# TJUMMG/OCPG

Hardware: AMD Instinct MI355X
Metric: clips/sec fwd+bwd (5x384x640, R101) (higher is better)
Workload: dtype bf16

## Files before the change

include/ocpg_hip.h:

```cpp
#ifndef OCPG_HIP_H
#define OCPG_HIP_H
#include <stdint.h>

#ifdef __cplusplus
extern "C" {
#endif

int ocpg_msda_fwd_f32(const float* value, const int64_t* shapes, const int64_t* level_start,
                      const float* loc, const float* attn,
                      int N, int S, int M, int D, int L, int Lq, int P,
                      float* out, const int64_t* shapes_host, void* stream);
int ocpg_msda_fwd_f64(const double* value, const int64_t* shapes, const int64_t* level_start,
                      const double* loc, const double* attn,
                      int N, int S, int M, int D, int L, int Lq, int P,
                      double* out, void* stream);

int ocpg_msda_bwd_f32(const float* value, const int64_t* shapes, const int64_t* level_start,
                      const float* loc, const float* attn, const float* grad_out,
                      int N, int S, int M, int D, int L, int Lq, int P,
                      float* grad_value, float* grad_loc, float* grad_attn,
                      const int64_t* shapes_host, void* stream);
int ocpg_msda_bwd_value_f32(const float* loc, const float* attn, const float* grad_out,
                            int N, int S, int M, int D, int L, int Lq, int P,
                            float* grad_value, const int64_t* shapes_host, void* stream);
int ocpg_msda_bwd_locattn_f32(const float* value, const int64_t* shapes, const int64_t* level_start,
                              const float* loc, const float* attn, const float* grad_out,
                              int N, int S, int M, int D, int L, int Lq, int P,
                              float* grad_loc, float* grad_attn, void* stream);
int ocpg_msda_fused_fwd_f32(const float* value, const int64_t* shapes, const int64_t* level_start,
                            const float* qproj, const float* ref,
                            int N, int S, int M, int D, int L, int Lq, int P,
                            float* out, float* loc_out, float* attn_out, void* stream);
int ocpg_msda_fused_bwd_qproj_f32(const float* value, const int64_t* shapes, const int64_t* level_start,
                                  const float* loc, const float* attn, const float* grad_out,
                                  int N, int S, int M, int D, int L, int Lq, int P,
                                  float* grad_qproj, void* stream);
int ocpg_msda_bwd_value_sel_f32(const float* loc, const float* attn, const float* grad_out,
                                int N, int S, int M, int D, int L, int Lq, int P,
                                float* grad_value, const int64_t* shapes_host, int* sel_state, void* stream);
int ocpg_msda_bwd_f64(const double* value, const int64_t* shapes, const int64_t* level_start,
                      const double* loc, const double* attn, const double* grad_out,
                      int N, int S, int M, int D, int L, int Lq, int P,
                      double* grad_value, double* grad_loc, double* grad_attn, void* stream);

int ocpg_msda_fwd_h16(const void* value, const int64_t* shapes, const int64_t* level_start,
                      const float* loc, const float* attn,
                      int N, int S, int M, int D, int L, int Lq, int P,
                      void* out, const int64_t* shapes_host, int dtype, void* stream);
int ocpg_msda_bwd_h16(const void* value, const int64_t* shapes, const int64_t* level_start,
                      const float* loc, const float* attn, const void* grad_out,
                      int N, int S, int M, int D, int L, int Lq, int P,
                      float* grad_value, float* grad_loc, float* grad_attn,
                      const int64_t* shapes_host, int* sel_state, int dtype, void* stream);
int ocpg_msda_bwd_value_h16(const float* loc, const float* attn, const void* grad_out,
                            int N, int S, int M, int D, int L, int Lq, int P,
                            float* grad_value, const int64_t* shapes_host, int* sel_state, int dtype, void* stream);
int ocpg_msda_bwd_locattn_h16(const void* value, const int64_t* shapes, const int64_t* level_start,
                              const float* loc, const float* attn, const void* grad_out,
                              int N, int S, int M, int D, int L, int Lq, int P,
                              float* grad_loc, float* grad_attn, int dtype, void* stream);
int ocpg_msda_fused_fwd_h16(const void* value, const int64_t* shapes, const int64_t* level_start,
                            const float* qproj, const float* ref,
                            int N, int S, int M, int D, int L, int Lq, int P,
                            void* out, float* loc_out, float* attn_out, int dtype, void* stream);
int ocpg_msda_fused_bwd_qproj_h16(const void* value, const int64_t* shapes, const int64_t* level_start,
                                  const float* loc, const float* attn, const void* grad_out,
                                  int N, int S, int M, int D, int L, int Lq, int P,
                                  float* grad_qproj, int dtype, void* stream);

int ocpg_bn_act_fwd(const void* x, const float* scale, const float* shift, const void* skip, void* y,
                    long long n_outer, int C, long long inner, int relu, int dtype, void* stream);
int ocpg_bn_act_bwd(const void* gy, const void* y, const float* scale, void* gx, void* gskip,
                    long long n_outer, int C, long long inner, int relu, int dtype, void* stream);

int ocpg_gemm_dgrad_bn_tile(long long M, int N, int K);
int ocpg_gemm_dgrad_bn(const void* a, const void* w, const void* c, const void* mask, const float* scale, void* out, void* out_skip,
                       long long M, int N, int K, int dtype, int tile, void* stream);

int ocpg_win_attn_fwd(const void* qkv, const float* biasT, const int* region, float scale, int BW, int NW, int N, int H,
                      int head_dim, void* out, float* lse, int dtype, void* stream);
int ocpg_win_attn_bwd(const void* qkv, const float* bias, const float* biasT, const int* region, float scale, int BW, int NW,
                      int N, int H, int head_dim, const void* out, const void* dout, const float* lse, void* dqkv, float* Dbuf,
                      float* dbiasT, int dtype, void* stream);

int ocpg_win_attn_bwd_mfma(const void* qkv, const float* bias, const float* biasT, const int* region, float scale, int BW, int NW, int N,
                           int H, int head_dim, const void* out, const void* dout, const float* lse, void* dqkv, float* Dbuf, void* dS,
                           int dtype, void* stream);

int ocpg_win_attn_dtable_supported(int N, int head_dim, int dtype, int T);
int ocpg_win_attn_bwd_mfma_dtable(const void* qkv, const float* bias, const float* biasT, const int* region, float scale, int BW, int NW,
                                  int N, int H, int head_dim, const void* out, const void* dout, const float* lse, void* dqkv, float* Dbuf,
                                  const int* tok_code, int code_off, int T, float* partials, float* dtable, int dtype, void* stream);

int ocpg_dynmask_fwd_f32(const float* feats, const float* params, const float* refpix, int BT, int Q, int C, int H, int W,
                         int stride, float* out, float* pre1, void* stream);

int ocpg_dynmask_bwd_pre_f32(const float* dout, const float* pre1, const float* params, int BT, int Q, int C, int H, int W,
                             int stride, float* dpre, float* part, float* w0d, void* stream);
int ocpg_dynmask_bwd_fin_f32(const float* part, const float* params, const float* refpix, const float* dw0, int BT, int Q, int C,
                             int H, int W, float* dparams, float* dref, void* stream);

int ocpg_im2col3x3_nhwc(const void* x, int N, int H, int W, int C, int stride, int dil, void* cols, int dtype, void* stream);
int ocpg_col2im3x3_nhwc(const void* dcols, int N, int H, int W, int C, int stride, int dil, void* dx, int dtype, void* stream);

int ocpg_conv3x3_mfma_fwd(const void* x, const void* w, const float* scale, const float* bias, int relu, int N, int H, int W,
                          int Cin, int Cout, int stride, void* y, void* stream);
int ocpg_conv3x3_mfma_fwd_cols(const void* x, const void* w, const float* scale, const float* bias, int relu, int N, int H, int W, int Cin,
                               int Cout, int stride, void* y, void* cols, void* stream);
int ocpg_conv3x3_mfma_dgrad(const void* dy, const void* wT, int N, int H, int W, int Cin, int Cout, int stride, void* dx,
                            void* stream);
int ocpg_conv3x3_mfma_dgrad_masked(const void* dy, const void* wT, const void* mask_y, const float* scale, int N, int H, int W, int Cin,
                                   int Cout, int stride, void* dx, void* stream);
int ocpg_conv3x3_mfma_dgrad_w(const void* dy, const void* w, const void* mask_y, const float* scale, int N, int H, int W, int Cin, int Cout,
                              int stride, void* dx, void* stream);
int ocpg_conv3x3_mfma_body_splits(long long M, int ncols, int kchannels);
int ocpg_conv3x3_mfma_fwd_bn_splitk(const void* x, const void* w, const float* scale, const float* shift, int relu, int N, int H, int W, int Cin,
                                    int Cout, int stride, int splits, float* part, void* y, void* stream);
int ocpg_conv3x3_mfma_dgrad_w_splitk(const void* dy, const void* w, const void* mask_y, const float* scale, int N, int H, int W, int Cin,
                                     int Cout, int stride, int splits, float* part, void* dx, void* stream);
int ocpg_conv3x3_mfma_wgrad_splits(int N, int H, int W, int Cin, int Cout, int stride);
int ocpg_conv3x3_mfma_wgrad(const void* gz, const void* x, int N, int H, int W, int Cin, int Cout, int stride, void* part, void* stream);
int ocpg_conv3x3_mfma_fwd_cols_h16(const void* x, const void* w, const float* scale, const float* bias, int relu, int N, int H, int W, int Cin,
                                   int Cout, int stride, void* y, void* cols, int dtype, void* stream);
int ocpg_conv3x3_mfma_dgrad_w_h16(const void* dy, const void* w, const void* mask_y, const float* scale, int N, int H, int W, int Cin, int Cout,
                                  int stride, void* dx, int dtype, void* stream);
int ocpg_conv3x3_mfma_wgrad_h16(const void* gz, const void* x, int N, int H, int W, int Cin, int Cout, int stride, void* part, int dtype,
// ... 165 lines not shown
```

ocpg_amd/_lib.py:

```python
import ctypes
import os

import torch

_HERE = os.path.dirname(os.path.abspath(__file__))
LIB_PATH = os.environ.get("OCPG_HIP_LIB") or os.path.join(_HERE, "lib", "libocpg_hip.so")
_lib = None

_i64p = ctypes.c_void_p
_vp = ctypes.c_void_p
_int = ctypes.c_int

SIGNATURES = {
    "ocpg_msda_fwd_f32": [_vp, _i64p, _i64p, _vp, _vp] + [_int] * 7 + [_vp, _vp, _vp],
    "ocpg_msda_fwd_f64": [_vp, _i64p, _i64p, _vp, _vp] + [_int] * 7 + [_vp, _vp],
    "ocpg_msda_bwd_f32": [_vp, _i64p, _i64p, _vp, _vp, _vp] + [_int] * 7 + [_vp, _vp, _vp, _vp, _vp],
    "ocpg_msda_bwd_value_f32": [_vp, _vp, _vp] + [_int] * 7 + [_vp, _vp, _vp],
    "ocpg_msda_fused_fwd_f32": [_vp, _i64p, _i64p, _vp, _vp] + [_int] * 7 + [_vp, _vp, _vp, _vp],
    "ocpg_msda_fused_bwd_qproj_f32": [_vp, _i64p, _i64p, _vp, _vp, _vp] + [_int] * 7 + [_vp, _vp],
    "ocpg_msda_bwd_value_sel_f32": [_vp, _vp, _vp] + [_int] * 7 + [_vp, _vp, _vp, _vp],
    "ocpg_msda_bwd_locattn_f32": [_vp, _i64p, _i64p, _vp, _vp, _vp] + [_int] * 7 + [_vp, _vp, _vp],
    "ocpg_msda_bwd_f64": [_vp, _i64p, _i64p, _vp, _vp, _vp] + [_int] * 7 + [_vp, _vp, _vp, _vp],
    "ocpg_msda_fwd_h16": [_vp, _i64p, _i64p, _vp, _vp] + [_int] * 7 + [_vp, _vp, _int, _vp],
    "ocpg_msda_bwd_h16": [_vp, _i64p, _i64p, _vp, _vp, _vp] + [_int] * 7 + [_vp, _vp, _vp, _vp, _vp, _int, _vp],
    "ocpg_msda_bwd_value_h16": [_vp, _vp, _vp] + [_int] * 7 + [_vp, _vp, _vp, _int, _vp],
    "ocpg_msda_bwd_locattn_h16": [_vp, _i64p, _i64p, _vp, _vp, _vp] + [_int] * 7 + [_vp, _vp, _int, _vp],
    "ocpg_msda_fused_fwd_h16": [_vp, _i64p, _i64p, _vp, _vp] + [_int] * 7 + [_vp, _vp, _vp, _int, _vp],
    "ocpg_msda_fused_bwd_qproj_h16": [_vp, _i64p, _i64p, _vp, _vp, _vp] + [_int] * 7 + [_vp, _int, _vp],
    "ocpg_bn_act_fwd": [_vp, _vp, _vp, _vp, _vp, ctypes.c_longlong, _int, ctypes.c_longlong, _int, _int, _vp],
    "ocpg_bn_act_bwd": [_vp, _vp, _vp, _vp, _vp, ctypes.c_longlong, _int, ctypes.c_longlong, _int, _int, _vp],
    "ocpg_gemm_dgrad_bn_tile": [ctypes.c_longlong, _int, _int],
    "ocpg_gemm_dgrad_bn": [_vp] * 7 + [ctypes.c_longlong, _int, _int, _int, _int, _vp],
    "ocpg_dynmask_fwd_f32": [_vp, _vp, _vp] + [_int] * 6 + [_vp, _vp, _vp],
    "ocpg_dynmask_bwd_pre_f32": [_vp, _vp, _vp] + [_int] * 6 + [_vp, _vp, _vp, _vp],
    "ocpg_dynmask_bwd_fin_f32": [_vp, _vp, _vp, _vp] + [_int] * 5 + [_vp, _vp, _vp],
    "ocpg_conv3x3_mfma_fwd": [_vp, _vp, _vp, _vp] + [_int] * 7 + [_vp, _vp],
    "ocpg_conv3x3_mfma_fwd_cols": [_vp, _vp, _vp, _vp] + [_int] * 7 + [_vp, _vp, _vp],
    "ocpg_conv3x3_mfma_dgrad": [_vp, _vp] + [_int] * 6 + [_vp, _vp],
    "ocpg_conv3x3_mfma_dgrad_masked": [_vp, _vp, _vp, _vp] + [_int] * 6 + [_vp, _vp],
    "ocpg_conv3x3_mfma_dgrad_w": [_vp, _vp, _vp, _vp] + [_int] * 6 + [_vp, _vp],
    "ocpg_conv3x3_mfma_splits": [_int] * 6,
    "ocpg_conv3x3_mfma_wgrad_splits": [_int] * 6,
    "ocpg_conv3x3_mfma_body_splits": [ctypes.c_longlong, _int, _int],
    "ocpg_conv3x3_mfma_fwd_bn_splitk": [_vp, _vp, _vp, _vp] + [_int] * 8 + [_vp, _vp, _vp],
    "ocpg_conv3x3_mfma_dgrad_w_splitk": [_vp, _vp, _vp, _vp] + [_int] * 7 + [_vp, _vp, _vp],
    "ocpg_conv3x3_mfma_wgrad": [_vp, _vp] + [_int] * 6 + [_vp, _vp],
    "ocpg_conv3x3_mfma_fwd_cols_h16": [_vp, _vp, _vp, _vp] + [_int] * 7 + [_vp, _vp, _int, _vp],
    "ocpg_conv3x3_mfma_dgrad_w_h16": [_vp, _vp, _vp, _vp] + [_int] * 6 + [_vp, _int, _vp],
    "ocpg_conv3x3_mfma_wgrad_h16": [_vp, _vp] + [_int] * 6 + [_vp, _int, _vp],
    "ocpg_conv3x3_mfma_dgrad_w_s2": [_vp, _vp, _vp, _vp] + [_int] * 6 + [_vp, _vp],
    "ocpg_conv3x3_mfma_dgrad_w_s2_h16": [_vp, _vp, _vp, _vp] + [_int] * 6 + [_vp, _int, _vp],
    "ocpg_conv3x3_mfma_fwd_splitk": [_vp, _vp, _vp] + [_int] * 7 + [_vp, _vp, _int, _vp, _vp],
    "ocpg_conv3x3_mfma_fwd_splitk_h16": [_vp, _vp, _vp] + [_int] * 7 + [_vp, _vp, _int, _vp, _int, _vp],
    "ocpg_gemm": [_vp, _vp, _vp, _vp] + [_int] * 4 + [ctypes.c_longlong] * 10 + [ctypes.c_float, ctypes.c_float, _vp],
    "ocpg_gemm_plans": [],
    "ocpg_gemm_tuned": [_vp],
    "ocpg_gemm_tune_rejected": [],
    "ocpg_gemm_set_tuning": [_int],
    "ocpg_gemm_export_picks": [_vp, ctypes.c_longlong],
    "ocpg_gemm_import_picks": [_vp, ctypes.c_longlong],
    "ocpg_window_means3x3_fwd": [_vp, ctypes.c_longlong, _int, _int, _int, _vp, _vp],
    "ocpg_window_means3x3_bwd": [_vp, ctypes.c_longlong, _int, _int, _vp, _vp],
    "ocpg_window_sums3x3_cl_bands": [_int],
    "ocpg_window_sums3x3_cl": [_vp, _int, _int, _int, _int, _int, _vp, _vp],
    "ocpg_window_means3x3_bwd_cl": [_vp, _int, _int, _int, _int, _vp, _vp, _vp],
    "ocpg_mso_conv3x3": [_vp, _int, _int, _vp, _int, _vp, _vp, _int, _vp, _int, _vp, _vp, _int] + [_int] * 6 + [_vp],
    "ocpg_mso_wgrad_rows": [_int] * 4,
    "ocpg_mso_wgrad": [_vp, _int, _int, _vp, _vp, _vp] + [_int] * 8 + [_vp],
    "ocpg_bilinear_nhwc_fwd": [_vp] + [_int] * 6 + [_vp, _vp],
    "ocpg_bilinear_nhwc_bwd": [_vp] + [_int] * 6 + [_vp, _vp],
    "ocpg_small_linear_fwd": [_vp, _int, _vp, _vp, _int, _int, _int, _int, _vp, _vp],
    "ocpg_small_linear_bwd": [_vp, _int, _vp, _int, _vp, _vp, _int, _int, _int, _vp, _vp, _vp, _vp],
    "ocpg_small_linear_fwd_h16": [_vp, _int, _vp, _vp, _int, _int, _int, _int, _vp, _int, _vp],
    "ocpg_small_linear_bwd_h16": [_vp, _int, _vp, _int, _vp, _vp, _int, _int, _int, _vp, _vp, _vp, _int, _vp],
    "ocpg_small_linear_f32_fwd": [_vp, _vp, _vp, _int, _int, _int, _vp, _vp],
    "ocpg_small_linear_f32_bwd": [_vp, _vp, _vp, _int, _int, _int, _vp, _vp, _vp, _vp],
    "ocpg_layernorm_blocks": [ctypes.c_longlong],
    "ocpg_groupnorm_cl_work": [ctypes.c_longlong, _int, _int, _int],
    "ocpg_groupnorm_cl_fwd": [_vp, _int, _vp, _vp, ctypes.c_longlong, _int, _int, _int, ctypes.c_float, _vp, _vp, _vp, _vp, _vp],
    "ocpg_groupnorm_cl_bwd": [_vp, _vp, _int, _vp, _vp, _vp, ctypes.c_longlong, _int, _int, _int, _vp, _vp, _vp, _vp],
    "ocpg_groupnorm_cl2cl_fwd": [_vp, _int, _vp, _vp, ctypes.c_longlong, _int, _int, _int, ctypes.c_float, _vp, _vp, _vp, _vp, _vp],
    "ocpg_groupnorm_cl2cl_bwd": [_vp, _vp, _int, _vp, _vp, _vp, ctypes.c_longlong, _int, _int, _int, _vp, _vp, _vp, _vp],
    "ocpg_layernorm_fwd": [_vp, _int, _vp, _vp, ctypes.c_longlong, _int, ctypes.c_float, _vp, _int, _vp, _vp, _vp],
    "ocpg_layernorm_bwd": [_vp, _int, _vp, _int, _vp, _vp, _vp, ctypes.c_longlong, _int, _vp, _int, _vp, _vp, _vp],
    "ocpg_gather_rows_bwd": [_vp, _vp, _vp, _int, _int, _vp, _vp],
    "ocpg_relpos_bias_fwd": [_vp, _vp, _int, ctypes.c_longlong, _int, _vp, _vp, _vp],
    "ocpg_relpos_bias_bwd": [_vp, _vp, _vp, _int, _int, _int, _int, _vp, _vp],
    "ocpg_gather_rows_pad": [_vp, _vp] + [ctypes.c_longlong] * 4 + [_vp, _vp],
    "ocpg_graph_replace_memsets": [_vp, _vp],
    "ocpg_graph_stats": [_vp, _vp],
    "ocpg_graph_memcpy_nodes": [_vp, _vp, _int],
    "ocpg_gemm_bn_act": [_vp] * 6 + [_int, _int] + [ctypes.c_longlong] * 3 + [_vp],
    "ocpg_levelset_fwd_f32": [_vp] * 3 + [_int] * 6 + [_vp] * 4,
    "ocpg_levelset_bwd_f32": [_vp] * 5 + [_int] * 6 + [_vp] * 3,
    "ocpg_proj_fwd_f32": [_vp] * 5 + [_int] * 5 + [_vp] * 5,
    "ocpg_proj_bwd_f32": [_vp] * 9 + [_int] * 5 + [_vp] * 4,
    "ocpg_matcher_cost_f32": [_vp] * 3 + [ctypes.c_longlong] * 4 + [_vp] * 4 + [_int] * 7 + [ctypes.c_float] * 5 + [_vp] * 4,
    "ocpg_dropout_add_ln_fwd": [_vp] * 4 + [ctypes.c_longlong, _int, ctypes.c_float, ctypes.c_float, ctypes.c_ulonglong, ctypes.c_ulonglong, _vp, _int]
                               + [_vp] * 4,
    "ocpg_dropout_add_ln_bwd": [_vp] * 6 + [ctypes.c_longlong, _int, ctypes.c_float, ctypes.c_ulonglong, ctypes.c_ulonglong, _vp, _int] + [_vp] * 4,
    "ocpg_dropout_add_ln_bwd_slots": [ctypes.c_longlong],
    "ocpg_bias_relu_dropout_fwd": [_vp, _vp, ctypes.c_longlong, _int, ctypes.c_float, ctypes.c_ulonglong, ctypes.c_ulonglong, _vp, _int, _vp, _vp],
    "ocpg_bias_relu_dropout_bwd": [_vp, _vp, ctypes.c_longlong, _int, ctypes.c_float, _int, _vp, _vp, _vp],
    "ocpg_bias_relu_dropout_bwd_slots": [ctypes.c_longlong, _int, _int],
    "ocpg_multi_cast": [_vp] * 4 + [_int, ctypes.c_longlong, _int, _int, _vp],
# ... 148 lines not shown
```

ocpg_amd/models/ops/functions/ms_deform_attn_func.py:

```python
import ctypes

import torch
from torch.autograd import Function
from torch.autograd.function import once_differentiable

from ...._lib import check, lib, require_gpu, stream_ptr


_TIMING = {"on": False, "events": []}


def enable_kernel_timing(on=True):
    _TIMING["on"] = on
    _TIMING["events"] = []


def collect_kernel_timing():
    torch.cuda.synchronize()
    out = {}
    for key, e0, e1 in _TIMING["events"]:
        d = out.setdefault(key, {"ms": 0.0, "n": 0})
        d["ms"] += e0.elapsed_time(e1)
        d["n"] += 1
    _TIMING["events"] = []
# ... 187 lines not shown
                    loc = (ref.view(N, Lq, 1, L, 1, 2) + off.reshape(N, Lq, M, L, P, 2)).contiguous()
                    rc = lib().ocpg_msda_fwd_h16(value.data_ptr(), shapes.data_ptr(), level_start.data_ptr(), loc.data_ptr(), attn.data_ptr(),
                                                 N, S, M, D, L, Lq, P, out.data_ptr(), None, code, stream_ptr())
                check(rc, "ocpg_msda_fused_fwd_h16")
            else:
                check(lib().ocpg_msda_fused_fwd_f32(value.data_ptr(), shapes.data_ptr(), level_start.data_ptr(), qproj.data_ptr(), ref.data_ptr(),
                                                    N, S, M, D, L, Lq, P, out.data_ptr(), loc.data_ptr(), attn.data_ptr(), stream_ptr()),
                      "ocpg_msda_fused_fwd")
        ctx.save_for_backward(value, shapes, level_start, loc, attn)
        ctx.shapes_host = getattr(shapes, "_ocpg_host", None)
        ctx.sel_state = sel_state
        ctx.qshape = qproj.shape
        ctx.mark_non_differentiable(loc, attn)
        return out, loc, attn

    @staticmethod
    @once_differentiable
    def backward(ctx, grad_output, _gloc, _gattn):
        value, shapes, level_start, loc, attn = ctx.saved_tensors
        N, S, M, D = value.shape
        _, Lq, _, L, P, _ = loc.shape
        go = grad_output.contiguous()
        hs = ctx.shapes_host if ctx.shapes_host is not None else _host_shapes(shapes)
        if value.dtype in _H16:
            return MSDeformAttnFusedFunction._backward_h16(ctx, value, shapes, level_start, loc, attn, go, hs)
        grad_value = torch.zeros_like(value)
        grad_q = torch.empty(ctx.qshape, dtype=value.dtype, device=value.device)
        L_ = lib()
        with torch.cuda.device(value.device):
            with _timed("bwd_enc_value"):
                args = (loc.data_ptr(), attn.data_ptr(), go.data_ptr(), N, S, M, D, L, Lq, P, grad_value.data_ptr(), ctypes.c_void_p(hs.data_ptr()))
                if ctx.sel_state is not None:
                    rc = L_.ocpg_msda_bwd_value_sel_f32(*args, ctx.sel_state.data_ptr(), stream_ptr())
                else:
                    rc = L_.ocpg_msda_bwd_value_f32(*args, stream_ptr())
            if rc == -2000:
                grad_value.zero_()
                gl, ga = torch.empty_like(loc), torch.empty_like(attn)
                check(L_.ocpg_msda_bwd_f32(value.data_ptr(), shapes.data_ptr(), level_start.data_ptr(), loc.data_ptr(), attn.data_ptr(), go.data_ptr(),
                                           N, S, M, D, L, Lq, P, grad_value.data_ptr(), gl.data_ptr(), ga.data_ptr(), ctypes.c_void_p(hs.data_ptr()),
                                           stream_ptr()), "ocpg_msda_bwd")
                glogit = attn.view(N, Lq, M, L * P) * (ga.view(N, Lq, M, L * P) - (attn * ga).view(N, Lq, M, L * P).sum(-1, keepdim=True))
                grad_q = torch.cat([gl.reshape(N, Lq, -1), glogit.reshape(N, Lq, -1)], -1)
                return grad_value, None, None, grad_q, None, None, None, None
            check(rc, "ocpg_msda_bwd_value")
            with _timed("bwd_enc_locattn"):
                check(L_.ocpg_msda_fused_bwd_qproj_f32(value.data_ptr(), shapes.data_ptr(), level_start.data_ptr(), loc.data_ptr(), attn.data_ptr(),
                                                       go.data_ptr(), N, S, M, D, L, Lq, P, grad_q.data_ptr(), stream_ptr()), "ocpg_msda_fused_bwd_qproj")
        return grad_value, None, None, grad_q, None, None, None, None

    @staticmethod
    def _backward_h16(ctx, value, shapes, level_start, loc, attn, go, hs):
        N, S, M, D = value.shape
        _, Lq, _, L, P, _ = loc.shape
        if go.dtype != value.dtype:
            raise RuntimeError(f"MSDeformAttnFusedFunction: grad_output must have value's dtype {value.dtype} (got {go.dtype})")
        code = _H16[value.dtype]
        grad_value = torch.zeros(value.shape, dtype=torch.float32, device=value.device)
        grad_q = torch.empty(ctx.qshape, dtype=torch.float32, device=value.device)
        sel = ctx.sel_state.data_ptr() if ctx.sel_state is not None else None
        hsp = ctypes.c_void_p(hs.data_ptr())
        L_ = lib()
        with torch.cuda.device(value.device):
            with _timed("bwd_enc_value"):
                rc = L_.ocpg_msda_bwd_value_h16(loc.data_ptr(), attn.data_ptr(), go.data_ptr(), N, S, M, D, L, Lq, P, grad_value.data_ptr(), hsp, sel,
                                                code, stream_ptr())
            if rc == 0:
                with _timed("bwd_enc_locattn"):
                    rc = L_.ocpg_msda_fused_bwd_qproj_h16(value.data_ptr(), shapes.data_ptr(), level_start.data_ptr(), loc.data_ptr(), attn.data_ptr(),
                                                          go.data_ptr(), N, S, M, D, L, Lq, P, grad_q.data_ptr(), code, stream_ptr())
                if rc == -2000:
                    grad_value.zero_()
            if rc == -2000:
                gl, ga = torch.empty_like(loc), torch.empty_like(attn)
                with _timed("bwd_enc"):
                    check(L_.ocpg_msda_bwd_h16(value.data_ptr(), shapes.data_ptr(), level_start.data_ptr(), loc.data_ptr(), attn.data_ptr(), go.data_ptr(),
                                               N, S, M, D, L, Lq, P, grad_value.data_ptr(), gl.data_ptr(), ga.data_ptr(), hsp, sel, code, stream_ptr()),
                          "ocpg_msda_bwd_h16")
                glogit = attn.view(N, Lq, M, L * P) * (ga.view(N, Lq, M, L * P) - (attn * ga).view(N, Lq, M, L * P).sum(-1, keepdim=True))
                grad_q = torch.cat([gl.reshape(N, Lq, -1), glogit.reshape(N, Lq, -1)], -1).view(ctx.qshape)
            else:
                check(rc, "ocpg_msda_fused_bwd_h16")
        return grad_value.to(value.dtype), None, None, grad_q, None, None, None, None
```

ocpg_amd/models/ops/modules/ms_deform_attn.py:

```python
import math
import os
import warnings

import torch
import torch.nn.functional as F
from torch import nn

from ... import amp_cache
from ...amp_cache import TokenLinear, linear
from ....util.misc import memo
from ..functions import MSDeformAttnFunction
from ..functions.ms_deform_attn_func import MSDeformAttnFusedFunction


FUSED_FRONT = os.environ.get("OCPG_MSDA_FUSED_FRONT", "1") != "0"
FUSED_FRONT_H16 = os.environ.get("OCPG_MSDA_FUSED_FRONT_H16", "0") != "0"
SELECT_PATH = os.environ.get("OCPG_MSDA_SELECT", "1") != "0"
MERGED_QUERY_PROJ = True


_UNSET = object()
_VALUE_DTYPES = {"fp32": None, "bf16": torch.bfloat16, "fp16": torch.float16, "autocast": "autocast"}


def resolve_value_dtype(word=None):
    src = "msda_value_dtype"
    if word is None:
        word, src = os.environ.get("OCPG_MSDA_VALUE_DTYPE") or "fp32", "OCPG_MSDA_VALUE_DTYPE"
    if word not in _VALUE_DTYPES:
        raise ValueError(f"{src} must be one of {sorted(_VALUE_DTYPES)}, not {word!r}")
    return _VALUE_DTYPES[word]


def _is_power_of_2(n):
    if not isinstance(n, int) or n < 0:
        raise ValueError(f"invalid input for _is_power_of_2: {n} (type: {type(n)})")
    return n != 0 and (n & (n - 1)) == 0


class MSDeformAttn(nn.Module):
    def __init__(self, d_model=256, n_levels=4, n_heads=8, n_points=4, value_dtype=None):
        super().__init__()
        if d_model % n_heads:
            raise ValueError(f"d_model must be divisible by n_heads, but got {d_model} and {n_heads}")
        if not _is_power_of_2(d_model // n_heads):
            warnings.warn("d_model // n_heads should be a power of 2 (the fast HIP kernel needs it; others take the generic kernel)")
        self.im2col_step = 64
        self.d_model, self.n_levels, self.n_heads, self.n_points = d_model, n_levels, n_heads, n_points
        self.sampling_offsets = TokenLinear(d_model, n_heads * n_levels * n_points * 2)
        self.attention_weights = TokenLinear(d_model, n_heads * n_levels * n_points)
        self.value_proj = TokenLinear(d_model, d_model)
        self.output_proj = TokenLinear(d_model, d_model)
        self.register_buffer("_sel_state", torch.zeros(8, dtype=torch.int32), persistent=False)
        self.set_value_dtype(value_dtype)
        self._reset_parameters()

    def set_value_dtype(self, value_dtype):
        if value_dtype not in (None, torch.bfloat16, torch.float16, "autocast"):
            raise ValueError(f"value_dtype must be None, torch.bfloat16, torch.float16 or 'autocast', not {value_dtype!r}")
        self.value_dtype = value_dtype
        if value_dtype is not None:
            amp_cache.register(self, self.value_proj.weight, self.value_proj.bias, self.output_proj.weight, self.output_proj.bias)
        else:
            self.__dict__.pop("_amp_cache_extra", None)

    def active_value_dtype(self, x):
        vd = self.value_dtype
        if vd is None or not x.is_cuda:
            return None
        if vd == "autocast":
            vd = torch.get_autocast_dtype("cuda") if torch.is_autocast_enabled("cuda") else None
            return vd if vd in (torch.bfloat16, torch.float16) else None
        return vd

    @staticmethod
    def _linear16(x, lin, dt):
        w, b = amp_cache.lookup(lin.weight), amp_cache.lookup(lin.bias)
        return linear(x.to(dt), w.to(dt), b.to(dt))

    def _reset_parameters(self):
        nn.init.zeros_(self.sampling_offsets.weight)
        theta = torch.arange(self.n_heads, dtype=torch.float32) * (2.0 * math.pi / self.n_heads)
        ring = torch.stack([theta.cos(), theta.sin()], -1)
        ring = ring / ring.abs().max(-1, keepdim=True)[0]
        ring = ring.view(self.n_heads, 1, 1, 2).repeat(1, self.n_levels, self.n_points, 1)
        ring = ring * torch.arange(1, self.n_points + 1, dtype=torch.float32).view(1, 1, -1, 1)
        with torch.no_grad():
            self.sampling_offsets.bias = nn.Parameter(ring.reshape(-1))
        nn.init.zeros_(self.attention_weights.weight)
        nn.init.zeros_(self.attention_weights.bias)
        nn.init.xavier_uniform_(self.value_proj.weight)
        nn.init.zeros_(self.value_proj.bias)
        nn.init.xavier_uniform_(self.output_proj.weight)
        nn.init.zeros_(self.output_proj.bias)

    def forward(self, query, reference_points, input_flatten, input_spatial_shapes, input_level_start_index,
                input_padding_mask=None, value_dtype=_UNSET):
        N, Lq, _ = query.shape
        vd = self.active_value_dtype(input_flatten) if value_dtype is _UNSET else value_dtype
        _, S, _ = input_flatten.shape
        M, L, P = self.n_heads, self.n_levels, self.n_points
        host = getattr(input_spatial_shapes, "_ocpg_host", None)
        if host is not None:
            assert int((host[:, 0] * host[:, 1]).sum()) == S
        else:
            assert (input_spatial_shapes[:, 0] * input_spatial_shapes[:, 1]).sum() == S

        value = self.value_proj(input_flatten) if vd is None else self._linear16(input_flatten, self.value_proj, vd)
        if input_padding_mask is not None:
            value = value.masked_fill(input_padding_mask[..., None], 0.0)
        value = value.view(N, S, M, self.d_model // M)
        if MERGED_QUERY_PROJ and query.is_cuda:
            n_off = M * L * P * 2
            so_w, so_b = self.sampling_offsets.weight, self.sampling_offsets.bias
            folded = reference_points.shape[-1] == 2 and host is not None
            if folded:
                key = ("msda_inv_wh", tuple(host.flatten().tolist()), M, P)
                inv = memo("msda", key, query.device, lambda: (1.0 / torch.stack([host[:, 1], host[:, 0]], -1).float())[None, :, None, :]
                           .expand(M, L, P, 2).reshape(-1).to(query.device))
                so_w, so_b = so_w * inv[:, None], so_b * inv
            both = linear(query, torch.cat([so_w, self.attention_weights.weight], 0), torch.cat([so_b, self.attention_weights.bias], 0))
            if ((FUSED_FRONT if vd is None else FUSED_FRONT_H16) and folded and Lq == S
                    and MSDeformAttnFusedFunction.supported(value, both, reference_points, L, P)):
                out, loc, weights = MSDeformAttnFusedFunction.apply(value.contiguous(), input_spatial_shapes, input_level_start_index, both,
                                                                    reference_points, L, P, self._sel_state if SELECT_PATH else None)
                return (self.output_proj(out) if vd is None else self._linear16(out, self.output_proj, vd)), loc, weights
            off2, logit2 = torch.split(both, [n_off, M * L * P], dim=-1)
            offsets = off2.view(N, Lq, M, L, P, 2)
            weights = F.softmax(logit2.view(N, Lq, M, L * P), -1).view(N, Lq, M, L, P)
        else:
            folded = False
            offsets = self.sampling_offsets(query).view(N, Lq, M, L, P, 2)
            weights = F.softmax(self.attention_weights(query).view(N, Lq, M, L * P), -1).view(N, Lq, M, L, P)
        if reference_points.shape[-1] == 2:
            if folded:
                loc = reference_points[:, :, None, :, None, :] + offsets
            else:
                wh = torch.stack([input_spatial_shapes[..., 1], input_spatial_shapes[..., 0]], -1)
                loc = reference_points[:, :, None, :, None, :] + offsets / wh[None, None, None, :, None, :]
        elif reference_points.shape[-1] == 4:
            loc = reference_points[:, :, None, :, None, :2] + offsets / P * reference_points[:, :, None, :, None, 2:] * 0.5
        else:
            raise ValueError(f"Last dim of reference_points must be 2 or 4, but get {reference_points.shape[-1]} instead.")
        loc_c = loc.contiguous()
        if SELECT_PATH and Lq == S and loc_c.is_cuda:
            loc_c._ocpg_sel = self._sel_state
        out = MSDeformAttnFunction.apply(value.contiguous(), input_spatial_shapes, input_level_start_index,
                                         loc_c, weights.contiguous(), self.im2col_step)
        return (self.output_proj(out) if vd is None else self._linear16(out, self.output_proj, vd)), loc, weights
```

Measured before the change: 61.39.

## Add sample-first MSDA path that samples raw source before value projection

Adds HIP kernels that bilinearly sample the unprojected source features and apply the value projection afterwards, per query and head. This is used for cross-attention (Lq != S) when queries are few relative to S. It avoids projecting and storing the full value tensor when only a small set of sampled points is needed. The backward pass recomputes the projected gradient per row and scatters source gradients with atomics, which adds extra per-row GEMV work and atomic contention. The path is on by default, but it uses the fp32 path only (vd None), so it may not trigger under bf16 autocast.

```diff
diff --git a/include/ocpg_hip.h b/include/ocpg_hip.h
--- a/include/ocpg_hip.h
+++ b/include/ocpg_hip.h
@@ -42,6 +42,17 @@
                       const double* loc, const double* attn, const double* grad_out,
                       int N, int S, int M, int D, int L, int Lq, int P,
                       double* grad_value, double* grad_loc, double* grad_attn, void* stream);
+
+int ocpg_msda_sf_fwd_f32(const float* src, const float* wv, const float* bv, const unsigned char* pad,
+                         const int64_t* shapes, const int64_t* level_start, const float* loc, const float* attn,
+                         int N, int S, int M, int D, int L, int Lq, int P,
+                         float* out, float* s, float* beta, void* stream);
+int ocpg_msda_sf_bwd_f32(const float* src, const float* wv, const float* bv, const unsigned char* pad,
+                         const int64_t* shapes, const int64_t* level_start, const float* loc, const float* attn,
+                         const float* grad_out, int N, int S, int M, int D, int L, int Lq, int P,
+                         float* grad_src, float* grad_loc, float* grad_attn, void* stream);
+int ocpg_msda_sf_bwd_params_f32(const float* grad_out, const float* s, const float* beta, int N, int M, int D, int Lq,
+                                float* grad_wv, float* grad_bv, void* stream);
 
 int ocpg_msda_fwd_h16(const void* value, const int64_t* shapes, const int64_t* level_start,
                       const float* loc, const float* attn,
diff --git a/ocpg_amd/_lib.py b/ocpg_amd/_lib.py
--- a/ocpg_amd/_lib.py
+++ b/ocpg_amd/_lib.py
@@ -21,6 +21,9 @@
     "ocpg_msda_bwd_value_sel_f32": [_vp, _vp, _vp] + [_int] * 7 + [_vp, _vp, _vp, _vp],
     "ocpg_msda_bwd_locattn_f32": [_vp, _i64p, _i64p, _vp, _vp, _vp] + [_int] * 7 + [_vp, _vp, _vp],
     "ocpg_msda_bwd_f64": [_vp, _i64p, _i64p, _vp, _vp, _vp] + [_int] * 7 + [_vp, _vp, _vp, _vp],
+    "ocpg_msda_sf_fwd_f32": [_vp, _vp, _vp, _vp, _i64p, _i64p, _vp, _vp] + [_int] * 7 + [_vp, _vp, _vp, _vp],
+    "ocpg_msda_sf_bwd_f32": [_vp, _vp, _vp, _vp, _i64p, _i64p, _vp, _vp, _vp] + [_int] * 7 + [_vp, _vp, _vp, _vp],
+    "ocpg_msda_sf_bwd_params_f32": [_vp, _vp, _vp] + [_int] * 4 + [_vp, _vp, _vp],
     "ocpg_msda_fwd_h16": [_vp, _i64p, _i64p, _vp, _vp] + [_int] * 7 + [_vp, _vp, _int, _vp],
     "ocpg_msda_bwd_h16": [_vp, _i64p, _i64p, _vp, _vp, _vp] + [_int] * 7 + [_vp, _vp, _vp, _vp, _vp, _int, _vp],
     "ocpg_msda_bwd_value_h16": [_vp, _vp, _vp] + [_int] * 7 + [_vp, _vp, _vp, _int, _vp],
diff --git a/ocpg_amd/csrc/msda_sample_first.hip b/ocpg_amd/csrc/msda_sample_first.hip
--- /dev/null
+++ b/ocpg_amd/csrc/msda_sample_first.hip
@@ -0,0 +1,391 @@
+#include <hip/hip_runtime.h>
+#include <stdint.h>
+
+#include "../../include/ocpg_hip.h"
+#include "msda_dev.h"
+
+namespace {
+
+constexpr int kMaxSamples = 64;
+constexpr int kMaxC = 1024;
+constexpr int kThreads = 256;
+
+using ocpg_dev::SampleRec;
+using ocpg_dev::make_sample;
+
+__device__ __forceinline__ void setup_samples(const int64_t* __restrict__ shapes, const int64_t* __restrict__ level_start,
+                                              const float* __restrict__ lrow, const float* __restrict__ arow,
+                                              const unsigned char* __restrict__ padn, int P, int NS, int C, SampleRec* recs) {
+  const int s = threadIdx.x;
+  if (s < NS) {
+    const int l = s / P;
+    const int H = (int)shapes[2 * l], W = (int)shapes[2 * l + 1];
+    SampleRec rec;
+    make_sample<float>(lrow[2 * s], lrow[2 * s + 1], arow[s], H, W, (int)level_start[l], C, rec);
+    if (padn && rec.mask) {
+      const int pix = rec.off00 / C;
+      const int dp[4] = {0, 1, W, W + 1};
+#pragma unroll
+      for (int k = 0; k < 4; ++k)
+        if ((rec.mask & (1 << k)) && padn[pix + dp[k]]) rec.mask &= ~(1 << k);
+    }
+    recs[s] = rec;
+  }
+}
+
+__device__ __forceinline__ float wave_sum(float v) {
+#pragma unroll
+  for (int o = 32; o > 0; o >>= 1) v += __shfl_xor(v, o, 64);
+  return v;
+}
+
+template <int CPT>
+__global__ __launch_bounds__(kThreads) void msda_sf_fwd(const float* __restrict__ src, const float* __restrict__ wv,
+                                                         const float* __restrict__ bv, const unsigned char* __restrict__ pad,
+                                                         const int64_t* __restrict__ shapes, const int64_t* __restrict__ level_start,
+                                                         const float* __restrict__ loc, const float* __restrict__ attn, int S, int M, int D,
+                                                         int L, int Lq, int P, float* __restrict__ out, float* __restrict__ s_out,
+                                                         float* __restrict__ beta_out) {
+  __shared__ SampleRec recs[kMaxSamples];
+  __shared__ float sv[kMaxC];
+  const int C = M * D, NS = L * P, T = blockDim.x, tid = threadIdx.x;
+  const long long row = blockIdx.x;
+  const int h = (int)(row % M);
+  const long long nq = row / M;
+  const long long n = nq / Lq;
+  setup_samples(shapes, level_start, loc + row * NS * 2, attn + row * NS, pad ? pad + n * S : nullptr, P, NS, C, recs);
+  __syncthreads();
+
+  int ch[CPT];
+#pragma unroll
+  for (int i = 0; i < CPT; ++i) ch[i] = min(tid + i * T, C - 1);
+  const float* sb = src + n * (long long)S * C;
+  float acc[CPT];
+#pragma unroll
+  for (int i = 0; i < CPT; ++i) acc[i] = 0.f;
+  float beta = 0.f;
+#pragma unroll 4
+  for (int s = 0; s < NS; ++s) {
+    const SampleRec rec = recs[s];
+    const float hy = 1.f - rec.ly, hx = 1.f - rec.lx;
+    const float w[4] = {hy * hx, hy * rec.lx, rec.ly * hx, rec.ly * rec.lx};
+    const int offs[4] = {0, C, rec.rowstride, rec.rowstride + C};
+    float v[4][CPT];
+#pragma unroll
+    for (int k = 0; k < 4; ++k) {
+      const bool ok = (rec.mask >> k) & 1;
+      const float* p = sb + (ok ? rec.off00 + offs[k] : 0);
+#pragma unroll
+      for (int i = 0; i < CPT; ++i) v[k][i] = p[ch[i]];
+    }
+    float wsum = 0.f;
+#pragma unroll
+    for (int k = 0; k < 4; ++k) {
+      const bool ok = (rec.mask >> k) & 1;
+      wsum += ok ? w[k] : 0.f;
+#pragma unroll
+      for (int i = 0; i < CPT; ++i) v[k][i] = ok ? v[k][i] : 0.f;
+    }
+#pragma unroll
+    for (int i = 0; i < CPT; ++i) acc[i] += (w[0] * v[0][i] + w[1] * v[1][i] + w[2] * v[2][i] + w[3] * v[3][i]) * rec.a;
+    beta += wsum * rec.a;
+  }
+#pragma unroll
+  for (int i = 0; i < CPT; ++i) {
+    const int c = tid + i * T;
+    if (c < C) {
+      sv[c] = acc[i];
+      s_out[row * C + c] = acc[i];
+    }
+  }
+  if (tid == 0) beta_out[row] = beta;
+  __syncthreads();
+  const int lane = tid & 63, wave = tid >> 6, nw = T >> 6;
+  for (int d = wave; d < D; d += nw) {
+    const float* wr = wv + (long long)(h * D + d) * C;
+    float p = 0.f;
+    for (int c = lane; c < C; c += 64) p += sv[c] * wr[c];
+    p = wave_sum(p);
+    if (lane == 0) out[nq * C + h * D + d] = p + (bv ? beta * bv[h * D + d] : 0.f);
+  }
+}
+
+template <int CPT, bool SCATTER>
+__global__ __launch_bounds__(kThreads) void msda_sf_bwd(const float* __restrict__ src, const float* __restrict__ wv,
+                                                         const float* __restrict__ bv, const unsigned char* __restrict__ pad,
+                                                         const int64_t* __restrict__ shapes, const int64_t* __restrict__ level_start,
+                                                         const float* __restrict__ loc, const float* __restrict__ attn,
+                                                         const float* __restrict__ gout, int S, int M, int D, int L, int Lq, int P,
+                                                         float* __restrict__ gsrc, float* __restrict__ gloc, float* __restrict__ gattn) {
+  __shared__ SampleRec recs[kMaxSamples];
+  __shared__ float red[kThreads / 64][kMaxSamples][3];
+  const int C = M * D, NS = L * P, T = blockDim.x, tid = threadIdx.x;
+  const long long row = blockIdx.x;
+  const int h = (int)(row % M);
+  const long long nq = row / M;
+  const long long n = nq / Lq;
+  setup_samples(shapes, level_start, loc + row * NS * 2, attn + row * NS, pad ? pad + n * S : nullptr, P, NS, C, recs);
+
+  int ch[CPT];
+#pragma unroll
+  for (int i = 0; i < CPT; ++i) ch[i] = min(tid + i * T, C - 1);
+  const float* go = gout + nq * C + h * D;
+  float t[CPT];
+#pragma unroll
+  for (int i = 0; i < CPT; ++i) t[i] = 0.f;
+  float gb = 0.f;
+#pragma unroll 8
+  for (int d = 0; d < D; ++d) {
+    const float g = go[d];
+    const float* wr = wv + (long long)(h * D + d) * C;
+#pragma unroll
+    for (int i = 0; i < CPT; ++i) t[i] += g * wr[ch[i]];
+    if (bv) gb += g * bv[h * D + d];
+  }
+#pragma unroll
+  for (int i = 0; i < CPT; ++i)
+    if (tid + i * T >= C) t[i] = 0.f;
+  __syncthreads();
+
+  const float* sb = src + n * (long long)S * C;
+  float* gs = SCATTER ? gsrc + n * (long long)S * C : nullptr;
+  const int lane = tid & 63, wave = tid >> 6, nw = T >> 6;
+  constexpr int GS = CPT == 1 ? 4 : (CPT == 2 ? 2 : 1);
+  for (int s0 = 0; s0 < NS; s0 += GS) {
+    SampleRec rec[GS];
+    float v[GS][4][CPT];
+#pragma unroll
+    for (int u = 0; u < GS; ++u) {
+      rec[u] = recs[min(s0 + u, NS - 1)];
+      if (s0 + u >= NS) rec[u].mask = 0;
+      const int offs[4] = {0, C, rec[u].rowstride, rec[u].rowstride + C};
+#pragma unroll
+      for (int k = 0; k < 4; ++k) {
+        const bool ok = (rec[u].mask >> k) & 1;
+        const float* p = sb + (ok ? rec[u].off00 + offs[k] : 0);
+#pragma unroll
+        for (int i = 0; i < CPT; ++i) v[u][k][i] = p[ch[i]];
+      }
+    }
+    float part[GS][3];
+#pragma unroll
+    for (int u = 0; u < GS; ++u) {
+      const float hy = 1.f - rec[u].ly, hx = 1.f - rec[u].lx;
+      const float w[4] = {hy * hx, hy * rec[u].lx, rec[u].ly * hx, rec[u].ly * rec[u].lx};
+      const float dyc[4] = {-hx, -rec[u].lx, hx, rec[u].lx};
+      const float dxc[4] = {-hy, hy, -rec[u].ly, rec[u].ly};
+      const int offs[4] = {0, C, rec[u].rowstride, rec[u].rowstride + C};
+      float pa = 0.f, px = 0.f, py = 0.f;
+#pragma unroll
+      for (int k = 0; k < 4; ++k) {
+        if ((rec[u].mask >> k) & 1) {
+#pragma unroll
+          for (int i = 0; i < CPT; ++i) {
+            const float tv = t[i] * v[u][k][i];
+            pa += w[k] * tv;
+            px += dxc[k] * tv;
+            py += dyc[k] * tv;
+            if constexpr (SCATTER) {
+              if (tid + i * T < C) atomicAdd(gs + rec[u].off00 + offs[k] + ch[i], w[k] * rec[u].a * t[i]);
+            }
+          }
+        }
+      }
+      part[u][0] = pa;
+      part[u][1] = px;
+      part[u][2] = py;
+    }
+#pragma unroll
+    for (int o = 32; o > 0; o >>= 1)
+#pragma unroll
+      for (int u = 0; u < GS; ++u)
+#pragma unroll
+        for (int c = 0; c < 3; ++c) part[u][c] += __shfl_xor(part[u][c], o, 64);
+    if (lane == 0) {
+#pragma unroll
+      for (int u = 0; u < GS; ++u)
+        if (s0 + u < NS) {
+          red[wave][s0 + u][0] = part[u][0];
+          red[wave][s0 + u][1] = part[u][1];
+          red[wave][s0 + u][2] = part[u][2];
+        }
+    }
+  }
+  __syncthreads();
+  if (tid < NS) {
+    const SampleRec rec = recs[tid];
+    float ga = 0.f, gx = 0.f, gy = 0.f;
+    if (rec.mask != 0) {
+      for (int u = 0; u < nw; ++u) {
+        ga += red[u][tid][0];
+        gx += red[u][tid][1];
+        gy += red[u][tid][2];
+      }
+      const float hy = 1.f - rec.ly, hx = 1.f - rec.lx;
+      const float w[4] = {hy * hx, hy * rec.lx, rec.ly * hx, rec.ly * rec.lx};
+      const float dyc[4] = {-hx, -rec.lx, hx, rec.lx};
+      const float dxc[4] = {-hy, hy, -rec.ly, rec.ly};
+      float ws = 0.f, xs = 0.f, ys = 0.f;
+#pragma unroll
+      for (int k = 0; k < 4; ++k)
+        if ((rec.mask >> k) & 1) {
+          ws += w[k];
+          xs += dxc[k];
+          ys += dyc[k];
+        }
+      ga += gb * ws;
+      gx = rec.W * rec.a * (gx + gb * xs);
+      gy = rec.H * rec.a * (gy + gb * ys);
+    }
+    gattn[row * NS + tid] = ga;
+    *reinterpret_cast<float2*>(gloc + (row * NS + tid) * 2) = make_float2(gx, gy);
+  }
+}
+
+template <int CPT>
+__global__ __launch_bounds__(kThreads) void msda_sf_bwd_params(const float* __restrict__ gout, const float* __restrict__ s_in,
+                                                                const float* __restrict__ beta_in, long long R, int M, int D,
+                                                                float* __restrict__ gwv, float* __restrict__ gbv) {
+  const int C = M * D, T = blockDim.x, tid = threadIdx.x;
+  const int o = blockIdx.x, h = o / D;
+  int ch[CPT];
+#pragma unroll
+  for (int i = 0; i < CPT; ++i) ch[i] = min(tid + i * T, C - 1);
+  float acc[CPT];
+#pragma unroll
+  for (int i = 0; i < CPT; ++i) acc[i] = 0.f;
+  float b = 0.f;
+#pragma unroll 4
+  for (long long r = 0; r < R; ++r) {
+    const float g = gout[r * C + o];
+    const float* sr = s_in + (r * M + h) * C;
+#pragma unroll
+    for (int i = 0; i < CPT; ++i) acc[i] += g * sr[ch[i]];
+    b += g * beta_in[r * M + h];
+  }
+#pragma unroll
+  for (int i = 0; i < CPT; ++i) {
+    const int c = tid + i * T;
+    if (c < C) gwv[(long long)o * C + c] = acc[i];
+  }
+  if (gbv && tid == 0) gbv[o] = b;
+}
+
+inline bool aligned_to(const void* p, uintptr_t a) { return (reinterpret_cast<uintptr_t>(p) & (a - 1)) == 0; }
+
+inline bool shape_ok(long long S, int M, int D, int L, int P) {
+  const long long C = (long long)M * D;
+  return C % 64 == 0 && C <= kMaxC && (long long)L * P <= kMaxSamples && S * C < (1LL << 31);
+}
+
+inline int launch_status() {
+  const hipError_t e = hipGetLastError();
+  return e == hipSuccess ? 0 : -(int)e;
+}
+
+inline int check_dims(int N, int S, int M, int D, int L, int Lq, int P) {
+  if (N < 0) return -1009;
+  if (S <= 0) return -1010;
+  if (M <= 0) return -1011;
+  if (D <= 0) return -1012;
+  if (L <= 0) return -1013;
+  if (Lq < 0) return -1014;
+  if (P <= 0) return -1015;
+  return 0;
+}
+
+#define SF_DISPATCH(CPT_, ...)        \
+  switch (CPT_) {                     \
+    case 1: SF_LAUNCH(1, __VA_ARGS__); break; \
+    case 2: SF_LAUNCH(2, __VA_ARGS__); break; \
+    case 3: SF_LAUNCH(3, __VA_ARGS__); break; \
+    default: SF_LAUNCH(4, __VA_ARGS__); break; \
+  }
+
+}
+
+extern "C" {
+
+int ocpg_msda_sf_fwd_f32(const float* src, const float* wv, const float* bv, const unsigned char* pad, const int64_t* shapes,
+                         const int64_t* level_start, const float* loc, const float* attn, int N, int S, int M, int D, int L, int Lq, int P,
+                         float* out, float* s, float* beta, void* stream) {
+  if (int e = check_dims(N, S, M, D, L, Lq, P)) return e;
+  if (!shape_ok(S, M, D, L, P)) return -2000;
+  const long long rows = (long long)N * Lq * M;
+  if (rows == 0) return 0;
+  if (!src) return -1001;
+  if (!wv) return -1002;
+  if (!shapes) return -1005;
+  if (!level_start) return -1006;
+  if (!loc) return -1007;
+  if (!attn) return -1008;
+  if (!out) return -1016;
+  if (!s) return -1017;
+  if (!beta) return -1018;
+  if (rows >= (1LL << 31)) return -2000;
+  if (!aligned_to(src, 4) || !aligned_to(wv, 4) || !aligned_to(bv, 4) || !aligned_to(shapes, 8) || !aligned_to(level_start, 8) ||
+      !aligned_to(loc, 4) || !aligned_to(attn, 4) || !aligned_to(out, 4) || !aligned_to(s, 4) || !aligned_to(beta, 4))
+    return -2000;
+  const int C = M * D, T = C < kThreads ? C : kThreads, cpt = (C + kThreads - 1) / kThreads;
+  hipStream_t st = (hipStream_t)stream;
+#define SF_LAUNCH(CPT_, ...) msda_sf_fwd<CPT_><<<(unsigned)rows, T, 0, st>>>(__VA_ARGS__)
+  SF_DISPATCH(cpt, src, wv, bv, pad, shapes, level_start, loc, attn, S, M, D, L, Lq, P, out, s, beta)
+#undef SF_LAUNCH
+  return launch_status();
+}
+
+int ocpg_msda_sf_bwd_f32(const float* src, const float* wv, const float* bv, const unsigned char* pad, const int64_t* shapes,
+                         const int64_t* level_start, const float* loc, const float* attn, const float* grad_out, int N, int S, int M,
+                         int D, int L, int Lq, int P, float* grad_src, float* grad_loc, float* grad_attn, void* stream) {
+  if (int e = check_dims(N, S, M, D, L, Lq, P)) return e - 1;
+  if (!shape_ok(S, M, D, L, P)) return -2000;
+  const long long rows = (long long)N * Lq * M;
+  if (rows == 0) return 0;
+  if (!src) return -1001;
+  if (!wv) return -1002;
+  if (!shapes) return -1005;
+  if (!level_start) return -1006;
+  if (!loc) return -1007;
+  if (!attn) return -1008;
+  if (!grad_out) return -1009;
+  if (!grad_loc) return -1018;
+  if (!grad_attn) return -1019;
+  if (rows >= (1LL << 31)) return -2000;
+  if (!aligned_to(src, 4) || !aligned_to(wv, 4) || !aligned_to(bv, 4) || !aligned_to(shapes, 8) || !aligned_to(level_start, 8) ||
+      !aligned_to(loc, 4) || !aligned_to(attn, 4) || !aligned_to(grad_out, 4) || !aligned_to(grad_src, 4) || !aligned_to(grad_loc, 8) ||
+      !aligned_to(grad_attn, 4))
+    return -2000;
+  const int C = M * D, T = C < kThreads ? C : kThreads, cpt = (C + kThreads - 1) / kThreads;
+  hipStream_t st = (hipStream_t)stream;
+#define SF_LAUNCH(CPT_, ...)                                                          \
+  if (grad_src) msda_sf_bwd<CPT_, true><<<(unsigned)rows, T, 0, st>>>(__VA_ARGS__);   \
+  else msda_sf_bwd<CPT_, false><<<(unsigned)rows, T, 0, st>>>(__VA_ARGS__)
+  SF_DISPATCH(cpt, src, wv, bv, pad, shapes, level_start, loc, attn, grad_out, S, M, D, L, Lq, P, grad_src, grad_loc, grad_attn)
+#undef SF_LAUNCH
+  return launch_status();
+}
+
+int ocpg_msda_sf_bwd_params_f32(const float* grad_out, const float* s, const float* beta, int N, int M, int D, int Lq, float* grad_wv,
+                                float* grad_bv, void* stream) {
+  if (N < 0) return -1004;
+  if (M <= 0) return -1005;
+  if (D <= 0) return -1006;
+  if (Lq < 0) return -1007;
+  if (!shape_ok(1, M, D, 1, 1)) return -2000;
+  if (!grad_wv) return -1008;
+  const long long R = (long long)N * Lq;
+  if (R > 0) {
+    if (!grad_out) return -1001;
+    if (!s) return -1002;
+    if (!beta) return -1003;
+  }
+  if (!aligned_to(grad_out, 4) || !aligned_to(s, 4) || !aligned_to(beta, 4) || !aligned_to(grad_wv, 4) || !aligned_to(grad_bv, 4)) return -2000;
+  const int C = M * D, T = C < kThreads ? C : kThreads, cpt = (C + kThreads - 1) / kThreads;
+  hipStream_t st = (hipStream_t)stream;
+#define SF_LAUNCH(CPT_, ...) msda_sf_bwd_params<CPT_><<<(unsigned)C, T, 0, st>>>(__VA_ARGS__)
+  SF_DISPATCH(cpt, grad_out, s, beta, R, M, D, grad_wv, grad_bv)
+#undef SF_LAUNCH
+  return launch_status();
+}
+
+}
diff --git a/ocpg_amd/models/ops/functions/ms_deform_attn_func.py b/ocpg_amd/models/ops/functions/ms_deform_attn_func.py
--- a/ocpg_amd/models/ops/functions/ms_deform_attn_func.py
+++ b/ocpg_amd/models/ops/functions/ms_deform_attn_func.py
@@ -293,3 +293,106 @@
             else:
                 check(rc, "ocpg_msda_fused_bwd_h16")
         return grad_value.to(value.dtype), None, None, grad_q, None, None, None, None
+
+
+class MSDeformAttnSampleFirstFunction(Function):
+
+    @staticmethod
+    def supported(src, wv, bv, loc, attn):
+        if not (src.is_cuda and src.dtype == wv.dtype == loc.dtype == attn.dtype == torch.float32 and (bv is None or bv.dtype == torch.float32)):
+            return False
+        N, S, C = src.shape
+        _, Lq, M, L, P, _ = loc.shape
+        return C % M == 0 and C % 64 == 0 and C <= 1024 and L * P <= 64 and S * C < 2 ** 31 and N * Lq * M < 2 ** 31
+
+    @staticmethod
+    def forward(ctx, src, wv, bv, pad, shapes, level_start, loc, attn):
+        for n, t in (("src", src), ("wv", wv), ("shapes", shapes), ("level_start", level_start), ("loc", loc), ("attn", attn)):
+            require_gpu(n, t)
+        if shapes.dtype != torch.int64 or level_start.dtype != torch.int64:
+            raise RuntimeError("MSDeformAttnSampleFirstFunction: spatial_shapes / level_start_index must be int64")
+        N, S, C = src.shape
+        _, Lq, M, L, P, _ = loc.shape
+        D = C // M
+        src, wv, loc, attn = src.contiguous(), wv.contiguous(), loc.contiguous(), attn.contiguous()
+        bv = None if bv is None else bv.contiguous()
+        if pad is not None:
+            pad = pad.contiguous()
+            pad = pad.view(torch.uint8) if pad.dtype == torch.bool else pad.to(torch.uint8)
+        out = torch.empty((N, Lq, C), dtype=torch.float32, device=src.device)
+        s = torch.empty((N, Lq, M, C), dtype=torch.float32, device=src.device)
+        beta = torch.empty((N, Lq, M), dtype=torch.float32, device=src.device)
+        with torch.cuda.device(src.device), _timed("fwd_dec"):
+            check(lib().ocpg_msda_sf_fwd_f32(src.data_ptr(), wv.data_ptr(), bv.data_ptr() if bv is not None else None,
+                                             pad.data_ptr() if pad is not None else None, shapes.data_ptr(), level_start.data_ptr(),
+                                             loc.data_ptr(), attn.data_ptr(), N, S, M, D, L, Lq, P, out.data_ptr(), s.data_ptr(), beta.data_ptr(),
+                                             stream_ptr()), "ocpg_msda_sf_fwd_f32")
+        ctx.save_for_backward(src, wv, bv, pad, shapes, level_start, loc, attn, s, beta)
+        return out
+
+    @staticmethod
+    @once_differentiable
+    def backward(ctx, grad_output):
+        src, wv, bv, pad, shapes, level_start, loc, attn, s, beta = ctx.saved_tensors
+        return _sample_first_backward(ctx, grad_output, src, wv, bv, pad, shapes, level_start, loc, attn, s, beta)
+
+
+def _sample_first_backward(ctx, grad_output, src, wv, bv, pad, shapes, level_start, loc, attn, s, beta):
+    N, S, C = src.shape
+    _, Lq, M, L, P, _ = loc.shape
+    D = C // M
+    go = grad_output.contiguous()
+    need_src, need_wv, need_bv = ctx.needs_input_grad[0], ctx.needs_input_grad[1], bv is not None and ctx.needs_input_grad[2]
+    need_loc, need_attn = ctx.needs_input_grad[6], ctx.needs_input_grad[7]
+    grad_src = grad_loc = grad_attn = grad_wv = grad_bv = None
+    p = lambda t: t.data_ptr() if t is not None else None
+    with torch.cuda.device(src.device), _timed("bwd_dec"):
+        if need_src or need_loc or need_attn:
+            grad_src = torch.zeros_like(src) if need_src else None
+            grad_loc, grad_attn = torch.empty_like(loc), torch.empty_like(attn)
+            check(lib().ocpg_msda_sf_bwd_f32(src.data_ptr(), wv.data_ptr(), p(bv), p(pad), shapes.data_ptr(), level_start.data_ptr(),
+                                             loc.data_ptr(), attn.data_ptr(), go.data_ptr(), N, S, M, D, L, Lq, P,
+                                             p(grad_src), grad_loc.data_ptr(), grad_attn.data_ptr(), stream_ptr()), "ocpg_msda_sf_bwd_f32")
+        if need_wv or need_bv:
+            if s is None:
+                out = torch.empty((N, Lq, C), dtype=torch.float32, device=src.device)
+                s = torch.empty((N, Lq, M, C), dtype=torch.float32, device=src.device)
+                beta = torch.empty((N, Lq, M), dtype=torch.float32, device=src.device)
+                check(lib().ocpg_msda_sf_fwd_f32(src.data_ptr(), wv.data_ptr(), p(bv), p(pad), shapes.data_ptr(), level_start.data_ptr(),
+                                                 loc.data_ptr(), attn.data_ptr(), N, S, M, D, L, Lq, P, out.data_ptr(), s.data_ptr(),
+                                                 beta.data_ptr(), stream_ptr()), "ocpg_msda_sf_fwd_f32")
+            grad_wv = torch.empty_like(wv)
+            grad_bv = torch.empty_like(bv) if need_bv else None
+            check(lib().ocpg_msda_sf_bwd_params_f32(go.data_ptr(), s.data_ptr(), beta.data_ptr(), N, M, D, Lq, grad_wv.data_ptr(),
+                                                    p(grad_bv), stream_ptr()), "ocpg_msda_sf_bwd_params_f32")
+    return (grad_src, grad_wv if need_wv else None, grad_bv, None, None, None, grad_loc if need_loc else None,
+            grad_attn if need_attn else None)
+
+
+class MSDeformAttnSampleFirstBackwardFunction(Function):
+
+    supported = staticmethod(MSDeformAttnSampleFirstFunction.supported)
+
+    @staticmethod
+    def forward(ctx, src, wv, bv, pad, shapes, level_start, loc, attn):
+        from ...amp_cache import linear
+        for n, t in (("src", src), ("wv", wv), ("shapes", shapes), ("level_start", level_start), ("loc", loc), ("attn", attn)):
+            require_gpu(n, t)
+        N, S, C = src.shape
+        M = loc.shape[2]
+        src, wv, loc, attn = src.contiguous(), wv.contiguous(), loc.contiguous(), attn.contiguous()
+        bv = None if bv is None else bv.contiguous()
+        with torch.enable_grad():
+            value = linear(src.detach(), wv, bv).detach()
+        if pad is not None:
+            value = value.masked_fill(pad[..., None], 0.0)
+            pad = pad.contiguous()
+            pad = pad.view(torch.uint8) if pad.dtype == torch.bool else pad.to(torch.uint8)
+        out = ms_deform_attn_forward(value.view(N, S, M, C // M), shapes, level_start, loc, attn)
+        ctx.save_for_backward(src, wv, bv, pad, shapes, level_start, loc, attn)
+        return out
+
+    @staticmethod
+    @once_differentiable
+    def backward(ctx, grad_output):
+        return _sample_first_backward(ctx, grad_output, *ctx.saved_tensors, None, None)
diff --git a/ocpg_amd/models/ops/modules/ms_deform_attn.py b/ocpg_amd/models/ops/modules/ms_deform_attn.py
--- a/ocpg_amd/models/ops/modules/ms_deform_attn.py
+++ b/ocpg_amd/models/ops/modules/ms_deform_attn.py
@@ -10,12 +10,30 @@
 from ...amp_cache import TokenLinear, linear
 from ....util.misc import memo
 from ..functions import MSDeformAttnFunction
-from ..functions.ms_deform_attn_func import MSDeformAttnFusedFunction
+from ..functions.ms_deform_attn_func import (MSDeformAttnFusedFunction, MSDeformAttnSampleFirstBackwardFunction,
+                                              MSDeformAttnSampleFirstFunction)
 
 
 FUSED_FRONT = os.environ.get("OCPG_MSDA_FUSED_FRONT", "1") != "0"
 FUSED_FRONT_H16 = os.environ.get("OCPG_MSDA_FUSED_FRONT_H16", "0") != "0"
 SELECT_PATH = os.environ.get("OCPG_MSDA_SELECT", "1") != "0"
+
+
+def sample_first_mode(word):
+    if word not in ("0", "1", "force"):
+        raise ValueError(f"OCPG_MSDA_SAMPLE_FIRST must be one of '0', '1', 'force', not {word!r}")
+    return word
+
+
+SAMPLE_FIRST = sample_first_mode(os.environ.get("OCPG_MSDA_SAMPLE_FIRST", "1"))
+SAMPLE_FIRST_FWD = os.environ.get("OCPG_MSDA_SAMPLE_FIRST_FWD", "0") != "0"
+SAMPLE_FIRST_MAX_RATIO = 0.251
+
+
+def sample_first_wanted(N, S, M, Lq, L, P):
+    return Lq != S and N * S >= amp_cache.TOKEN_LINEAR_MIN_ROWS and 4 * Lq * L * P <= SAMPLE_FIRST_MAX_RATIO * S
+
+
 MERGED_QUERY_PROJ = True
 
 
@@ -106,10 +124,15 @@
         else:
             assert (input_spatial_shapes[:, 0] * input_spatial_shapes[:, 1]).sum() == S
 
-        value = self.value_proj(input_flatten) if vd is None else self._linear16(input_flatten, self.value_proj, vd)
-        if input_padding_mask is not None:
-            value = value.masked_fill(input_padding_mask[..., None], 0.0)
-        value = value.view(N, S, M, self.d_model // M)
+        def make_value():
+            value = self.value_proj(input_flatten) if vd is None else self._linear16(input_flatten, self.value_proj, vd)
+            if input_padding_mask is not None:
+                value = value.masked_fill(input_padding_mask[..., None], 0.0)
+            return value.view(N, S, M, self.d_model // M)
+
+        sample_first = (vd is None and input_flatten.is_cuda and Lq != S
+                        and (SAMPLE_FIRST == "force" or (SAMPLE_FIRST == "1" and sample_first_wanted(N, S, M, Lq, L, P))))
+        value = None if sample_first else make_value()
         if MERGED_QUERY_PROJ and query.is_cuda:
             n_off = M * L * P * 2
             so_w, so_b = self.sampling_offsets.weight, self.sampling_offsets.bias
@@ -143,6 +166,14 @@
         else:
             raise ValueError(f"Last dim of reference_points must be 2 or 4, but get {reference_points.shape[-1]} instead.")
         loc_c = loc.contiguous()
+        if sample_first:
+            vp = self.value_proj
+            fn = MSDeformAttnSampleFirstFunction if SAMPLE_FIRST_FWD else MSDeformAttnSampleFirstBackwardFunction if torch.is_grad_enabled() else None
+            if fn is not None and fn.supported(input_flatten, vp.weight, vp.bias, loc_c, weights):
+                out = fn.apply(input_flatten, vp.weight, vp.bias, input_padding_mask, input_spatial_shapes, input_level_start_index, loc_c,
+                               weights.contiguous())
+                return self.output_proj(out), loc, weights
+            value = make_value()
         if SELECT_PATH and Lq == S and loc_c.is_cuda:
             loc_c._ocpg_sel = self._sel_state
         out = MSDeformAttnFunction.apply(value.contiguous(), input_spatial_shapes, input_level_start_index,
```

New measurement: 62.56 (median of 6 runs). 1.9% higher.
